# vinhisreal/YOLO-LitePi

Hardware: AMD Instinct MI355X
Metric: images/sec end-to-end (det+NMS+clf) 640x640 batch64 (higher is better)
Workload: dtype f16; 1 GPU; configs[2]: full det+NMS+ROI+ShuffleNetV2 pipeline, fp16, batch=64/GPU, 640x640, inputs resident in HBM; classifier=ShuffleNetV2 x1.0, 91 classes, seeded random weights, 64x64 ROIs, min_area=50, max_det=300, steps_in_flight=3, distinct_input_batches=4, global_batch=64, boxes_pre_area_filter_rank0=413

## Files before the change

yolo-litepi_amd/csrc/c2f_kernels.hip:

```cpp
#include "c2f.h"

#include <cstdlib>

namespace lp {

typedef _Float16 half_t;
typedef _Float16 half8 __attribute__((ext_vector_type(8)));
typedef _Float16 half4 __attribute__((ext_vector_type(4)));
typedef float floatx4 __attribute__((ext_vector_type(4)));
typedef uint32_t u32x4 __attribute__((ext_vector_type(4)));
typedef uint32_t u32x2 __attribute__((ext_vector_type(2)));

namespace {

constexpr int cdiv_c(int a, int b) { return (a + b - 1) / b; }
constexpr int min_c(int a, int b) { return a < b ? a : b; }
constexpr int max_c(int a, int b) { return a > b ? a : b; }
constexpr int deep_depth(int S, int NT, int PT, bool ldsw) {
  int d = 2;
  for (int t = 3; t <= 6 && t <= S; ++t)
    if ((t * (PT + (ldsw ? 0 : NT)) + (ldsw ? 2 * NT : 0) + NT * PT) * 4 <= 180) d = t;
  return d;
}

template <int C_, int NB_, int KA_, int KB_, bool UP_, int COUT_, int MODE_, int KS2_, int TH_ = 20, int NW_PERIMG = 8, bool AW_ = true, int WPS_ = 0,
          bool DEEP_ = false, int NWT_ = 0>
struct C2fCfg {
  static constexpr int C = C_, NB = NB_, KA = KA_, KB = KB_, COUT = COUT_, MODE = MODE_, KS2 = KS2_;
  static constexpr bool UP = UP_;
  static constexpr bool PERIMG = MODE_ >= 1;
  static constexpr bool XCV1 = MODE_ == -1;
  static constexpr int NW = MODE_ >= 1 ? NW_PERIMG : (NWT_ > 0 ? NWT_ : (C_ >= 32 ? 8 : 4));
  static constexpr int TH = TH_, TW = 20;
  static constexpr int F = PERIMG ? 1 : 2 * NB;
  static constexpr int LW = TW + 2 * F, LH = TH + 2 * F;
  static constexpr bool GK = C % 32 != 0 && C != 16;
  static constexpr bool DEEP = DEEP_ || GK || C == 96;
  static constexpr int PS = C % 16 != 0 ? 2 * C : 2 * C + 16;
  static constexpr bool Y01 = C == 16 && NB == 1 && MODE_ == 0;
  static constexpr int PS0 = Y01 ? 4 * C + 16 : PS;
  static constexpr int Y1OFF = Y01 ? 2 * C : 0;
  static constexpr int PLANE0 = LW * LH * PS0, PLANE = LW * LH * PS;
  static constexpr int XC = 2 * C;
  static constexpr int e_cv1 = PERIMG ? 0 : 2 * NB;
  static constexpr int e_a(int k) { return PERIMG ? 0 : 2 * (NB - k) - 1; }
  static constexpr int e_b(int k) { return PERIMG ? 0 : 2 * (NB - k) - 2; }
  static constexpr int npt(int e) { return cdiv_c((TH + 2 * e) * (TW + 2 * e), 16); }
  static constexpr int MAXT = (MODE_ >= 1 && NW_PERIMG == 4) ? 52 : 20;
  static constexpr int cap_pt(int nt, int pt) { return nt * pt > (nt == 3 ? 21 : MAXT) ? cdiv_c(pt, 2) : pt; }
  static constexpr bool W1_LDS = PERIMG;
  static constexpr int CT1 = 2 * C / 16, NT1 = W1_LDS ? CT1 : (CT1 % 3 == 0 ? 3 : min_c(CT1, 4)), CB1 = CT1 / NT1,
                       PT1 = W1_LDS ? 2 : cap_pt(NT1, cdiv_c(npt(e_cv1), NW / CB1));
  static constexpr int CTM = cdiv_c(C, 16), NTM = CTM % 3 == 0 ? 3 : min_c(CTM, 2), CBM = CTM / NTM;
  static constexpr int ptm(int e) { return cdiv_c(npt(e), NW / CBM); }
  static constexpr int CT2 = COUT / 16, NT2 = CT2 % 3 == 0 ? 3 : (CT2 >= 2 ? CT2 / 2 : 1), CB2 = CT2 / NT2, PT2 = cap_pt(NT2, cdiv_c(npt(0), NW / CB2));
  static constexpr int PT2W = cdiv_c(npt(0), NW / CB2);
  static constexpr int NTS = NTM, CBS = CBM, PTS = cdiv_c(npt(0), NW / CBS);
  static constexpr int WPS = WPS_ > 0 ? WPS_ : (NW == 4 && MODE_ >= 1 ? 1 : 2);
  static constexpr bool CV2_TAB = GK || (C == 16 && NB == 2);
  static constexpr bool CV2_LDS = C >= 32 || Y01 || CV2_TAB;
  static constexpr int K2G = Y01 ? 0 : (CV2_LDS ? NB * C : (2 + NB) * C);
  static constexpr bool AW = !PERIMG && AW_;
  static constexpr int c3_steps = GK ? cdiv_c(9 * (C / 8), 4) : (C >= 32 ? 9 * (C / 32) : 5);
  static constexpr int WB_CV1 = CT1 * cdiv_c(KA + KB, 32) * 1024, WB_M = CTM * c3_steps * 1024, WB_CV2 = CT2 * cdiv_c((2 + NB) * C, 32) * 1024;
  static constexpr int WSLOT = AW ? max_c(WB_CV1, max_c(WB_M, WB_CV2)) : 0;
  static constexpr int NT_S2 = XC / 16, PT_S2 = 2;
  static constexpr int WB_S2 = PERIMG ? NT_S2 * 9 * (KS2 / 32) * 1024 : 0;
  static constexpr int LDS_BYTES = max_c(PLANE0 + PLANE + 2 * WSLOT, WB_S2);
  static_assert(!W1_LDS || WB_CV1 <= PLANE, "cv1's fragments are staged in plane 1");
  static C2fShape shape() {
    C2fShape s;
    s.C = C; s.NB = NB; s.KA = KA; s.KB = KB; s.UP = UP ? 1 : 0; s.COUT = COUT; s.MODE = MODE; s.KS2 = KS2;
    return s;
  }
};

struct Ctx {
  int n, oy0, ox0, H, W;
  int lane, wave, g, sig, gam;
  int dbg;
  unsigned long long* st;
};
#define C2F_ISTAMP(k)                                          \
  if (cx.st && threadIdx.x == 0) {                             \
    __builtin_amdgcn_sched_barrier(0);                         \
    cx.st[(k)] = clock64();                                    \
    __builtin_amdgcn_sched_barrier(0);                         \
  }
struct Rg {
  int gy0, gx0, fy0, fx0, rh, rw, R;
  unsigned magic;
};

#define C2F_STAMP(k) \
  if (a.stamps && threadIdx.x == 0) a.stamps[(size_t)blockIdx.x * 16 + (k)] = ((k) == 0 || (k) == 15) ? wall_clock64() : clock64();

#define C2F_GLDS16(gptr, lptr)                                                                        \
  __builtin_amdgcn_global_load_lds((const void __attribute__((address_space(1)))*)(gptr),          \
                                   (void __attribute__((address_space(3)))*)(lptr), 16, 0, 0)

__device__ __forceinline__ void wg_sync() {
  asm volatile("s_waitcnt vmcnt(0) lgkmcnt(0)" ::: "memory");
  __builtin_amdgcn_s_barrier();
  asm volatile("" ::: "memory");
}

__device__ __forceinline__ floatx4 mma16(half8 a, half8 b, floatx4 c) { return __builtin_amdgcn_mfma_f32_16x16x32_f16(a, b, c, 0, 0, 0); }
__device__ __forceinline__ half8 as_h8(u32x4 v) { return __builtin_bit_cast(half8, v); }

__device__ __forceinline__ floatx4 silu4(floatx4 v, floatx4 b) {
  v = v + b;
  float nl2e = -1.4426950408889634f;
  asm("" : "+s"(nl2e));
  const floatx4 t = v * floatx4{nl2e, nl2e, nl2e, nl2e};
  floatx4 e;
#pragma unroll
  for (int i = 0; i < 4; ++i) e[i] = __builtin_amdgcn_exp2f(t[i]);
  e = e + 1.f;
#pragma unroll
  for (int i = 0; i < 4; ++i) e[i] = __builtin_amdgcn_rcpf(e[i]);
  return v * e;
}

template <class CFG> __device__ __forceinline__ Rg make_region(const Ctx& cx, int E) {
  Rg r;
  const int y0 = max(cx.oy0 - E, 0), y1 = min(cx.oy0 + CFG::TH + E, cx.H);
  const int x0 = max(cx.ox0 - E, 0), x1 = min(cx.ox0 + CFG::TW + E, cx.W);
// ... 33 lines not shown
      *reinterpret_cast<half8*>(dst + 16 * j) = q;
    }
  }
}
template <int NT> __device__ __forceinline__ void load_h(const char* src, half_t (&h)[4 * NT]) {
  if constexpr (NT == 1) {
    const half4 q = *reinterpret_cast<const half4*>(src);
#pragma unroll
    for (int i = 0; i < 4; ++i) h[i] = q[i];
  } else if constexpr (NT % 2 == 1) {
#pragma unroll
    for (int j = 0; j < NT; ++j) {
      const half4 q = *reinterpret_cast<const half4*>(src + 8 * j);
#pragma unroll
      for (int i = 0; i < 4; ++i) h[4 * j + i] = q[i];
    }
  } else {
#pragma unroll
    for (int j = 0; j < NT / 2; ++j) {
      const half8 q = *reinterpret_cast<const half8*>(src + 16 * j);
#pragma unroll
      for (int i = 0; i < 8; ++i) h[8 * j + i] = q[i];
    }
  }
}
template <int NT> __device__ __forceinline__ void to_half(const floatx4 (&v)[NT], half_t (&h)[4 * NT]) {
#pragma unroll
  for (int t = 0; t < NT; ++t)
#pragma unroll
    for (int r = 0; r < 4; ++r) h[4 * t + r] = (half_t)v[t][r];
}

template <int S, int DA, int DB, int NT, int PT, class LA, class LB, class FX>
__device__ __forceinline__ void kloop(floatx4 (&acc)[NT][PT], LA&& la, LB&& lb, FX&& fix) {
  half8 af[DA][NT], bf[DB][PT];
#pragma unroll
  for (int s = 0; s < DA - 1; ++s)
    if (s < S) la(s, af[s]);
#pragma unroll
  for (int s = 0; s < DB - 1; ++s)
    if (s < S) lb(s, bf[s]);
#pragma unroll
  for (int s = 0; s < S; ++s) {
    if (s + DA - 1 < S) la(s + DA - 1, af[(s + DA - 1) % DA]);
    if (s + DB - 1 < S) lb(s + DB - 1, bf[(s + DB - 1) % DB]);
    __builtin_amdgcn_sched_barrier(0);
    fix(s, bf[s % DB]);
#pragma unroll
    for (int t = 0; t < NT; ++t)
#pragma unroll
      for (int i = 0; i < PT; ++i) acc[t][i] = mma16(af[s % DA][t], bf[s % DB][i], acc[t][i]);
  }
}
struct NoFix {
  template <int PT> __device__ __forceinline__ void operator()(int, half8 (&)[PT]) const {}
};

template <bool LDSW> struct ASrc {
  const char* base;
  template <int NT> __device__ __forceinline__ void load(int off_bytes, int s, half8 (&af)[NT]) const {
#pragma unroll
    for (int t = 0; t < NT; ++t) af[t] = as_h8(*reinterpret_cast<const u32x4*>(base + off_bytes + (s * NT + t) * 1024));
  }
};
__device__ __forceinline__ void stage_weights(const Ctx& cx, const void* src, char* slot, int bytes, int nw) {
  const char* s = reinterpret_cast<const char*>(src) + cx.lane * 16;
  for (int p = cx.wave; p < (bytes >> 10); p += nw) C2F_GLDS16(s + p * 1024, slot + p * 1024);
}

template <class CFG, int NT, int CB, int PT, int KA, int KB, int KL0, int KL1, bool UP, bool LDSW, class EPI, int PSL0 = CFG::PS, int PSL1 = CFG::PS>
__device__ __forceinline__ void pw_phase(const Ctx& cx, const Rg& rg, const char* __restrict__ srcA, int pitchA, const char* __restrict__ srcB,
                                         int pitchB, const char* pl0, const char* pl1, const ASrc<LDSW>& wsrc, const float* __restrict__ bias,
                                         EPI&& epi, int stamp0 = -1) {
  static_assert(KA % 32 == 0 && KB % 8 == 0 && KL0 % 32 == 0 && KL1 % 16 == 0 && (KB % 32 == 0 || KL0 + KL1 == 0),
                "K segments: whole steps, except a tail of whole 8-channel groups at the very end (global srcB, or 16 channels of plane 1)");
  constexpr int SA = KA / 32, SB = cdiv_c(KB, 32), SL0 = KL0 / 32, SL1 = cdiv_c(KL1, 32), SG = SA + SB, S = SG + SL0 + SL1;
  const int tail_off = (4 * (SB - 1) + cx.gam < KB / 8) ? (SB - 1) * 64 : -cx.gam * 16;
  const int npt = (rg.R + 15) >> 4;
  const int nblk = ((npt + PT - 1) / PT) * CB;
  for (int blk = cx.wave; blk < nblk; blk += CFG::NW) {
    const int cb = blk % CB, pbk = blk / CB;
    unsigned offA[SA > 0 ? PT : 1], offB[SB > 0 ? PT : 1];
    int pb[SL0 + SL1 > 0 ? PT : 1];
#pragma unroll
    for (int i = 0; i < PT; ++i) {
      int p = (pbk * PT + i) * 16 + cx.sig;
      p = p < rg.R ? p : rg.R - 1;
      int py, px;
      pix_of(rg, p, py, px);
      const int gy = rg.gy0 + py, gx = rg.gx0 + px;
      if constexpr (SA > 0) {
        const int ya = UP ? (gy >> 1) : gy, xa = UP ? (gx >> 1) : gx;
        const int HA = UP ? (cx.H >> 1) : cx.H, WA = UP ? (cx.W >> 1) : cx.W;
        offA[i] = (unsigned)(((cx.n * HA + ya) * WA + xa) * pitchA) * 2u + (unsigned)cx.gam * 16u;
      }
      if constexpr (SB > 0) offB[i] = (unsigned)(((cx.n * cx.H + gy) * cx.W + gx) * pitchB) * 2u + (unsigned)cx.gam * 16u;
      if constexpr (SL0 + SL1 > 0) pb[i] = (rg.fy0 + py) * CFG::LW + rg.fx0 + px;
    }
    floatx4 acc[NT][PT];
#pragma unroll
    for (int t = 0; t < NT; ++t)
#pragma unroll
      for (int i = 0; i < PT; ++i) acc[t][i] = floatx4{0.f, 0.f, 0.f, 0.f};
    int woff = (cb * S * NT * 64 + cx.lane) * 16;
    asm volatile("" : "+v"(woff));
    floatx4 bv[NT];
#pragma unroll
    for (int t = 0; t < NT; ++t) bv[t] = *reinterpret_cast<const floatx4*>(bias + cb * 16 * NT + 4 * NT * cx.g + 4 * t);
    constexpr int DB = CFG::DEEP ? deep_depth(S, NT, PT, LDSW)
                                 : ((CFG::PERIMG && LDSW) ? min_c(S, 5) : (((NT * PT <= 20 && CFG::C >= 32) || (CFG::WPS == 1 && NT * PT <= 28)) ? 3 : 2));
    constexpr int DA = LDSW ? 2 : DB;
    if (stamp0 >= 0) { C2F_ISTAMP(stamp0) }
    kloop<S, DA, DB, NT, PT>(
        acc, [&](int s, half8(&af)[NT]) { wsrc.template load<NT>(woff, s, af); },
        [&](int s, half8(&bf)[PT]) {
#pragma unroll
          for (int i = 0; i < PT; ++i) {
            if (s < SA) bf[i] = as_h8(*reinterpret_cast<const u32x4*>(srcA + (size_t)offA[SA > 0 ? i : 0] + s * 64));
            else if (s < SG && KB % 32 != 0 && s == SG - 1) bf[i] = as_h8(*reinterpret_cast<const u32x4*>(srcB + (size_t)(offB[SB > 0 ? i : 0] + (unsigned)tail_off)));
            else if (s < SG) bf[i] = as_h8(*reinterpret_cast<const u32x4*>(srcB + (size_t)offB[SB > 0 ? i : 0] + (s - SA) * 64));
            else if (s < SG + SL0) bf[i] = as_h8(*reinterpret_cast<const u32x4*>(pl0 + pb[SL0 + SL1 > 0 ? i : 0] * PSL0 + cx.gam * 16 + (s - SG) * 64));
            else bf[i] = as_h8(*reinterpret_cast<const u32x4*>(pl1 + pb[SL0 + SL1 > 0 ? i : 0] * PSL1 + (KL1 % 32 ? (cx.gam & 1) : cx.gam) * 16 + (s - SG - SL0) * 64));
          }
        },
        NoFix{});
    if (stamp0 >= 0) { C2F_ISTAMP(stamp0 + 1) }
#pragma unroll
    for (int i = 0; i < PT; ++i) {
      const int p0 = (pbk * PT + i) * 16 + cx.sig;
      const bool ok = p0 < rg.R;
      const int p = ok ? p0 : rg.R - 1;
      int py, px;
      pix_of(rg, p, py, px);
      floatx4 v[NT];
#pragma unroll
      for (int t = 0; t < NT; ++t) v[t] = silu4(acc[t][i], bv[t]);
      epi(cb, ok, py, px, v);
    }
    if (stamp0 >= 0) { C2F_ISTAMP(stamp0 + 2) }
  }
}

template <class CFG, int NT, int CB, int PT, bool LDSW, class EPI>
__device__ __forceinline__ void pw_gk_phase(const Ctx& cx, const Rg& rg, const char* __restrict__ cat, int cat_pitch, const char* pl0, const char* pl1,
                                            const ASrc<LDSW>& wsrc, const float* __restrict__ bias, EPI&& epi, int stamp0 = -1) {
  constexpr int G0 = CFG::K2G / 8, GC = CFG::C / 8, GT = G0 + 2 * GC, S = cdiv_c(GT, 4), PS = CFG::PS;
  static_assert(CFG::PS0 == CFG::PS && G0 >= 1, "one pixel pitch for both planes; y0 comes from the concat buffer");
  int goff[S];
  const char* lbase[S];
  bool isg[S];
#pragma unroll
  for (int s = 0; s < S; ++s) {
    int q = 4 * s + cx.gam;
    q = q < GT ? q : GT - 1;
    isg[s] = q < G0;
    goff[s] = (q < G0 ? q : G0 - 1) * 16;
    const int ql = q < G0 ? 0 : q - G0;
    lbase[s] = ql < GC ? pl0 + ql * 16 : pl1 + (ql - GC) * 16;
  }
  const int npt = (rg.R + 15) >> 4;
  const int nblk = ((npt + PT - 1) / PT) * CB;
  for (int blk = cx.wave; blk < nblk; blk += CFG::NW) {
    const int cb = blk % CB, pbk = blk / CB;
    unsigned offB[PT];
    int pb[PT];
#pragma unroll
    for (int i = 0; i < PT; ++i) {
      int p = (pbk * PT + i) * 16 + cx.sig;
      p = p < rg.R ? p : rg.R - 1;
      int py, px;
      pix_of(rg, p, py, px);
      offB[i] = (unsigned)(((cx.n * cx.H + rg.gy0 + py) * cx.W + rg.gx0 + px) * cat_pitch) * 2u;
      pb[i] = ((rg.fy0 + py) * CFG::LW + rg.fx0 + px) * PS;
    }
    floatx4 acc[NT][PT];
#pragma unroll
    for (int t = 0; t < NT; ++t)
#pragma unroll
      for (int i = 0; i < PT; ++i) acc[t][i] = floatx4{0.f, 0.f, 0.f, 0.f};
    int woff = (cb * S * NT * 64 + cx.lane) * 16;
    asm volatile("" : "+v"(woff));
    floatx4 bv[NT];
#pragma unroll
    for (int t = 0; t < NT; ++t) bv[t] = *reinterpret_cast<const floatx4*>(bias + cb * 16 * NT + 4 * NT * cx.g + 4 * t);
    constexpr int DB = deep_depth(S, NT, PT, LDSW);
    constexpr int DA = LDSW ? 2 : DB;
    if (stamp0 >= 0) { C2F_ISTAMP(stamp0) }
    kloop<S, DA, DB, NT, PT>(
        acc, [&](int s, half8(&af)[NT]) { wsrc.template load<NT>(woff, s, af); },
        [&](int s, half8(&bf)[PT]) {
          const bool pure_g = 4 * s + 3 < G0, pure_l = 4 * s >= G0;
// ... 394 lines not shown
  char* WS = smem + CFG::PLANE0 + CFG::PLANE;
  Ctx cx;
  cx.lane = threadIdx.x & 63;
  cx.wave = __builtin_amdgcn_readfirstlane(threadIdx.x >> 6);
  cx.g = cx.lane >> 4;
  {
    const int col = cx.lane & 15;
    cx.sig = col < 4 ? 2 * col : (col < 12 ? 2 * (col - 4) + 1 : 2 * (col - 8));
    cx.gam = ((cx.g & 1) << 1) | (cx.g >> 1);
  }
  cx.n = blockIdx.x % a.N;
  const int tile = blockIdx.x / a.N;
  const int ty = tile / a.tiles_x, tx = tile - ty * a.tiles_x;
  cx.oy0 = ty * TH; cx.ox0 = tx * TW;
  cx.H = a.H; cx.W = a.W;
  cx.st = a.stamps ? a.stamps + (size_t)blockIdx.x * 16 : nullptr;
  cx.dbg = a.debug_store;
  C2F_STAMP(0)
  C2F_STAMP(1)

  auto wslot = [&](int q) { return WS + (q & 1) * CFG::WSLOT; };
  auto stage = [&](int q) {
    if constexpr (AW) {
      if (q == 0) { if constexpr (!CFG::XCV1) stage_weights(cx, a.w[C2F_W_CV1], wslot(0), CFG::WB_CV1, CFG::NW); }
      else if (q == 2 * NB + 1) stage_weights(cx, a.w[C2F_W_CV2], wslot(q), CFG::WB_CV2, CFG::NW);
      else if (q <= 2 * NB) stage_weights(cx, a.w[C2F_W_A0 + q - 1], wslot(q), CFG::WB_M, CFG::NW);
    }
  };
  auto wsrc = [&](int q, int widx) {
    return ASrc<AW>{AW ? wslot(q) : reinterpret_cast<const char*>(a.w[widx])};
  };
  stage(0);
  stage(1);
  const char* src1 = reinterpret_cast<const char*>(a.src1);
  char* cat = reinterpret_cast<char*>(a.cat);
  const bool dbg = (a.debug_store & 1) != 0;

  if constexpr (CFG::MODE >= 1) {
    stage_weights(cx, a.w[C2F_W_S2], smem, CFG::WB_S2, CFG::NW);
    const Rg rg = make_region<CFG>(cx, 0);
    char* xo = reinterpret_cast<char*>(a.x);
    wg_sync();
    c3s2_phase<CFG, CFG::NT_S2, 1, CFG::PT_S2, true>(cx, rg, reinterpret_cast<const char*>(a.s2_in), a.s2_pitch, ASrc<true>{smem}, a.b[C2F_W_S2],
                                                     [&](int cb, bool ok, int py, int px, const floatx4(&v)[CFG::NT_S2]) {
                                                       constexpr int NT = CFG::NT_S2;
                                                       const int chb = cb * 16 * NT + 4 * NT * cx.g;
                                                       half_t h[4 * NT];
                                                       to_half<NT>(v, h);
                                                       const int gpix = (cx.n * cx.H + rg.gy0 + py) * cx.W + rg.gx0 + px;
                                                       if (ok) store_h<NT>(xo + (size_t)((unsigned)gpix * (unsigned)a.x_pitch) * 2 + chb * 2, h);
                                                     });
    wg_sync();
  }
  {
    const bool interior = !CFG::PERIMG && cx.oy0 >= F && cx.ox0 >= F && cx.oy0 + TH + F <= a.H && cx.ox0 + TW + F <= a.W;
    if constexpr (CFG::W1_LDS) stage_weights(cx, a.w[C2F_W_CV1], P1, CFG::WB_CV1, CFG::NW);
    if (!interior) {
      constexpr int NCLR = CFG::W1_LDS ? CFG::PLANE0 : CFG::PLANE0 + CFG::PLANE;
      for (int i = threadIdx.x; i < NCLR / 16; i += CFG::NW * 64) reinterpret_cast<u32x4*>(smem)[i] = u32x4{0u, 0u, 0u, 0u};
    }
  }
  wg_sync();
  C2F_STAMP(2)

  if constexpr (CFG::XCV1) {
    const Rg rg = make_region<CFG>(cx, CFG::e_cv1);
    constexpr int CG = C / 8, NTHR = CFG::NW * 64, NPC = cdiv_c(LW * CFG::LH * CG, NTHR);
    u32x4 v[NPC];
    int dst[NPC];
#pragma unroll
    for (int j = 0; j < NPC; ++j) {
      const int it = threadIdx.x + j * NTHR;
      const int pix = it / CG, cg = it - pix * CG;
      const bool valid = pix < rg.R;
      int py, px;
      pix_of(rg, valid ? pix : rg.R - 1, py, px);
      const int gpix = (cx.n * cx.H + rg.gy0 + py) * cx.W + rg.gx0 + px;
      v[j] = *reinterpret_cast<const u32x4*>(cat + (size_t)((unsigned)gpix * (unsigned)a.cat_pitch) * 2 + C * 2 + cg * 16);
      dst[j] = valid ? ((rg.fy0 + py) * LW + rg.fx0 + px) * PS0 + Y1OFF + cg * 16 : -1;
    }
#pragma unroll
    for (int j = 0; j < NPC; ++j)
      if (dst[j] >= 0) *reinterpret_cast<u32x4*>(P0 + dst[j]) = v[j];
  } else {
    const Rg rg = make_region<CFG>(cx, CFG::e_cv1);
    pw_phase<CFG, CFG::NT1, CFG::CB1, CFG::PT1, CFG::KA, CFG::KB, 0, 0, CFG::UP, AW || CFG::W1_LDS>(
        cx, rg, reinterpret_cast<const char*>(a.src0), a.pitch0, src1, a.pitch1, nullptr, nullptr,
        ASrc < AW || CFG::W1_LDS > {CFG::W1_LDS ? P1 : (AW ? wslot(0) : reinterpret_cast<const char*>(a.w[C2F_W_CV1]))}, a.b[C2F_W_CV1],
        [&](int cb, bool ok, int py, int px, const floatx4(&v)[CFG::NT1]) {
          constexpr int NT = CFG::NT1;
          const int chb = cb * 16 * NT + 4 * NT * cx.g;
          half_t h[4 * NT];
          to_half<NT>(v, h);
          const int fy = rg.fy0 + py, fx = rg.fx0 + px;
          if (ok) {
            if (CFG::Y01) store_h<NT>(P0 + (fy * LW + fx) * PS0 + chb * 2, h);
            else if (chb >= C) store_h<NT>(P0 + (fy * LW + fx) * PS0 + (chb - C) * 2, h);
            if ((chb < CFG::K2G || dbg) && fy >= F && fy < F + TH && fx >= F && fx < F + TW) {
              const int gpix = (cx.n * cx.H + rg.gy0 + py) * cx.W + rg.gx0 + px;
              store_h<NT>(cat + (size_t)((unsigned)gpix * (unsigned)a.cat_pitch) * 2 + chb * 2, h);
            }
          }
        }, CFG::PERIMG ? -1 : 8);
  }
  wg_sync();
  if constexpr (CFG::W1_LDS) {
    for (int i = threadIdx.x; i < CFG::PLANE / 16; i += CFG::NW * 64) reinterpret_cast<u32x4*>(P1)[i] = u32x4{0u, 0u, 0u, 0u};
    lds_sync();
  }
  C2F_STAMP(3)

#pragma unroll
  for (int k = 0; k < NB; ++k) {
    stage(2 * k + 2);
    {
      const Rg rg = make_region<CFG>(cx, CFG::e_a(k));
      auto epi_a = [&](int cb, bool ok, int py, int px, const floatx4(&v)[CFG::NTM]) {
        constexpr int NT = CFG::NTM;
        const int chb = cb * 16 * NT + 4 * NT * cx.g;
        half_t h[4 * NT];
        to_half<NT>(v, h);
        if (ok && (C % 16 == 0 || chb < C)) store_h<NT>(P1 + ((rg.fy0 + py) * LW + rg.fx0 + px) * PS + chb * 2, h);
      };
      const ASrc<AW> wa = wsrc(2 * k + 1, C2F_W_A0 + 2 * k);
      const float* ba = a.b[C2F_W_A0 + 2 * k];
      if (k == 0) c3_phase<CFG, CFG::ptm(CFG::e_a(0)), false, AW, PS0, Y1OFF>(cx, rg, P0, wa, ba, epi_a);
      else c3_phase<CFG, CFG::ptm(CFG::e_a(NB - 1)), false, AW, PS0, Y1OFF>(cx, rg, P0, wa, ba, epi_a);
    }
    wg_sync();
    stage(2 * k + 3);
    {
      const Rg rg = make_region<CFG>(cx, CFG::e_b(k));
      const bool last = k == NB - 1;
      auto epi_b = [&](int cb, bool ok, int py, int px, const floatx4(&v)[CFG::NTM]) {
        constexpr int NT = CFG::NTM;
        const int chb0 = cb * 16 * NT + 4 * NT * cx.g;
        const bool real = C % 16 == 0 || chb0 < C;
        const int chb = real ? chb0 : 0;
        const int fy = rg.fy0 + py, fx = rg.fx0 + px;
        char* yp = P0 + (fy * LW + fx) * PS0 + Y1OFF + chb * 2;
        half_t r[4 * NT], h[4 * NT];
        load_h<NT>(yp, r);
#pragma unroll
        for (int t = 0; t < NT; ++t)
#pragma unroll
          for (int q = 0; q < 4; ++q) h[4 * t + q] = (half_t)((float)(half_t)v[t][q] + (float)r[4 * t + q]);
        if (ok && real) {
          if (!last) store_h<NT>(yp, h);
          else if (CFG::CV2_LDS) store_h<NT>(P1 + (fy * LW + fx) * PS + chb * 2, h);
          if (((2 + k) * C < CFG::K2G || dbg) && fy >= F && fy < F + TH && fx >= F && fx < F + TW) {
            const int gpix = (cx.n * cx.H + rg.gy0 + py) * cx.W + rg.gx0 + px;
            store_h<NT>(cat + (size_t)((unsigned)gpix * (unsigned)a.cat_pitch) * 2 + ((2 + k) * C + chb) * 2, h);
          }
        }
      };
      const ASrc<AW> wbk = wsrc(2 * k + 2, C2F_W_B0 + 2 * k);
      const float* bbk = a.b[C2F_W_B0 + 2 * k];
      if (k == 0 && NB > 1) c3_phase<CFG, CFG::ptm(CFG::e_b(0)), false, AW, PS, 0>(cx, rg, P1, wbk, bbk, epi_b);
// ... 439 lines not shown
      half_t h[4 * NT];
      to_half<NT>(v, h);
      const int chb = os * CFG::COUTW + cb * 16 * NT + 4 * NT * cx.g;
      const int gpix = (cx.n * cx.H + py) * cx.W + px;
      if (ok) store_h<NT>(out + (size_t)((unsigned)gpix * (unsigned)a.out2_pitch) * 2 + chb * 2, h);
    }
  }
}
typedef SpCfg<96, 192, 192, 2> SpCfgV2;

typedef C2fCfg<32, 1, 128, 64, true, 64, 0, 0> CfgNeck40;
typedef C2fCfg<16, 1, 64, 32, true, 32, 0, 0, 16> CfgNeck80;
typedef C2fCfg<32, 1, 0, 128, false, 64, 0, 0> CfgPan40;
typedef C2fCfg<64, 1, 0, 256, false, 128, 1, 64> CfgPan20;
typedef C2fCfg<64, 1, 0, 128, false, 128, 2, 64> CfgBb20;
typedef C2fCfg<16, 2, 0, 32, false, 32, 0, 0, 16> CfgBb80;
typedef C2fCfg<32, 2, 0, 64, false, 64, 0, 0> CfgBb40;
typedef C2fCfg<48, 1, 192, 96, true, 96, 0, 0, 20, 8, false> CfgV2Neck40;
typedef C2fCfg<48, 1, 0, 144, false, 96, 0, 0, 20, 8, false> CfgV2Pan40;
typedef C2fCfg<24, 1, 96, 48, true, 48, 0, 0, 16> CfgV2Neck80;
typedef C2fCfg<96, 1, 0, 192, false, 192, 0, 0, 10, 8, false> CfgV2Bb20;
typedef C2fCfg<96, 1, 0, 288, false, 192, 0, 0, 10, 8, false> CfgV2Pan20;
typedef C2fCfg<24, 2, 0, 48, false, 48, -1, 0, 20, 8, true, 0, false, 8> CfgV2Bb80x;
typedef C2fCfg<16, 2, 0, 32, false, 32, -1, 0, 16> CfgBb80x;
typedef C2fCfg<64, 1, 0, 256, false, 128, 0, 0, 10, 8, false> CfgPan20h;
typedef C2fCfg<64, 1, 0, 128, false, 128, 0, 0, 10, 8, false> CfgBb20h;
typedef C2fCfg<24, 2, 0, 48, false, 48, 0, 0, 20, 8, true, 0, false, 8> CfgV2Bb80;
typedef C2fCfg<48, 2, 0, 96, false, 96, 0, 0, 10, 8, false> CfgV2Bb40;

template <class CFG> struct CfgName;
#define C2F_NAME(T, s) \
  template <> struct CfgName<T> { static const char* get() { return s; } };
C2F_NAME(CfgNeck40, "c2f<32,1,up128+64>")
C2F_NAME(CfgNeck80, "c2f<16,1,up64+32>")
C2F_NAME(CfgPan40, "c2f<32,1,128>")
C2F_NAME(CfgPan20, "c2f<64,1,s2+256>")
C2F_NAME(CfgBb20, "c2f<64,1,s2+128,sppf>")
C2F_NAME(CfgBb80, "c2f<16,2,32>")
C2F_NAME(CfgBb40, "c2f<32,2,64>")
C2F_NAME(CfgV2Neck40, "c2f<48,1,up192+96>")
C2F_NAME(CfgV2Pan40, "c2f<48,1,144>")
C2F_NAME(CfgV2Neck80, "c2f<24,1,up96+48>")
C2F_NAME(CfgV2Bb20, "c2f<96,1,192>")
C2F_NAME(CfgV2Pan20, "c2f<96,1,288>")
C2F_NAME(CfgV2Bb80, "c2f<24,2,48>")
C2F_NAME(CfgBb80x, "c2f<16,2,y0y1>")
C2F_NAME(CfgV2Bb80x, "c2f<24,2,y0y1>")
C2F_NAME(CfgPan20h, "c2f<64,1,256>")
C2F_NAME(CfgBb20h, "c2f<64,1,128>")
C2F_NAME(CfgV2Bb40, "c2f<48,2,96>")

template <class CFG> size_t cfg_lds() { return (size_t)CFG::LDS_BYTES; }

template <class CFG> bool try_launch(const C2fShape& s, const C2fArgs& a, hipStream_t st) {
  if (!(s == CFG::shape())) return false;
  const size_t lds = cfg_lds<CFG>();
  set_max_dynamic_lds(reinterpret_cast<const void*>(&c2f_kernel<CFG>), (int)lds);
  const int grid = a.N * a.tiles_x * a.tiles_y;
  LP_LAUNCH(c2f_kernel<CFG>, dim3(grid), dim3(CFG::NW * 64), lds, st, a);
  return true;
}
struct CfgInfo { size_t lds; const char* name; bool perimg, gk, cv2_lds; int th, tw, nt1, ntm, nt2, nt_s2; };
template <class CFG> bool try_info(const C2fShape& s, CfgInfo& ci) {
  if (!(s == CFG::shape())) return false;
  ci.lds = cfg_lds<CFG>();
  ci.name = CfgName<CFG>::get();
  ci.perimg = CFG::PERIMG;
  ci.gk = CFG::GK;
  ci.cv2_lds = CFG::CV2_LDS;
  ci.th = CFG::TH; ci.tw = CFG::TW;
  ci.nt1 = CFG::NT1; ci.ntm = CFG::NTM; ci.nt2 = CFG::NT2; ci.nt_s2 = CFG::NT_S2;
  return true;
}
template <class F> bool for_each_cfg(F&& f) {
  return f.template operator()<CfgNeck40>() || f.template operator()<CfgNeck80>() || f.template operator()<CfgPan40>() ||
         f.template operator()<CfgPan20>() || f.template operator()<CfgBb20>() || f.template operator()<CfgBb80>() ||
         f.template operator()<CfgBb40>() || f.template operator()<CfgV2Neck40>() || f.template operator()<CfgV2Pan40>() ||
         f.template operator()<CfgV2Neck80>() || f.template operator()<CfgV2Bb20>() || f.template operator()<CfgV2Pan20>() ||
         f.template operator()<CfgV2Bb80>() || f.template operator()<CfgV2Bb40>() || f.template operator()<CfgPan20h>() ||
         f.template operator()<CfgBb20h>() || f.template operator()<CfgBb80x>() || f.template operator()<CfgV2Bb80x>();
}
struct InfoFn {
  const C2fShape& s; CfgInfo& ci;
  template <class CFG> bool operator()() const { return try_info<CFG>(s, ci); }
};
struct LaunchFn {
  const C2fShape& s; const C2fArgs& a; hipStream_t st;
  template <class CFG> bool operator()() const { return try_launch<CFG>(s, a, st); }
};
bool cfg_info(const C2fShape& s, CfgInfo& ci) { return for_each_cfg(InfoFn{s, ci}); }
bool cfg_enabled(const C2fShape& s, CfgInfo& ci) {
  if (!getenv("LITEPI_C2F_BB80") && s == CfgBb80::shape()) return false;
  if (!cfg_info(s, ci)) return false;
  if (const char* skip = getenv("LITEPI_C2F_SKIP")) {
    const std::string list = std::string(";") + skip + ";", key = std::string(";") + ci.name + ";";
    if (list.find(key) != std::string::npos) return false;
  }
  return true;
}

int gam_of(int g) { return ((g & 1) << 1) | (g >> 1); }

template <class KIDX>
void pack_phase(DevBuf& dst, const std::vector<float>& Wm, int cout, int ktot, int NT, int S, KIDX&& kidx) {
  LP_CHECK((int)Wm.size() == cout * ktot, LP_ERR_STATE, "c2f: weight matrix %zu != %d x %d", Wm.size(), cout, ktot);
  const int CB = (cout + 16 * NT - 1) / (16 * NT);
  std::vector<uint16_t> buf((size_t)CB * S * NT * 64 * 8, 0);
  for (int cb = 0; cb < CB; ++cb)
    for (int s = 0; s < S; ++s)
      for (int t = 0; t < NT; ++t)
        for (int lane = 0; lane < 64; ++lane) {
          const int g = lane >> 4, m = lane & 15, gm = m >> 2, r = m & 3;
          const int oc = cb * 16 * NT + gm * 4 * NT + t * 4 + r;
          const size_t f = ((((size_t)cb * S + s) * NT + t) * 64 + lane) * 8;
          if (oc >= cout) continue;
          for (int j = 0; j < 8; ++j) {
            const int k = kidx(s, g, j);
            if (k >= 0) buf[f + j] = f32_to_f16(Wm[(size_t)oc * ktot + k]);
          }
        }
  dst.alloc(buf.size() * 2, false);
  LP_HIP(hipMemcpy(dst.p, buf.data(), buf.size() * 2, hipMemcpyHostToDevice));
}
void put_bias(DevBuf& dst, const std::vector<float>* b, int cout) {
  std::vector<float> v(cout + 64, 0.f);
  if (b) {
    LP_CHECK((int)b->size() >= cout, LP_ERR_STATE, "c2f: bias vector too short");
    for (int c = 0; c < cout; ++c) v[c] = (*b)[c];
  }
  dst.alloc(v.size() * 4, false);
  LP_HIP(hipMemcpy(dst.p, v.data(), v.size() * 4, hipMemcpyHostToDevice));
}

}

static DevBuf g_stamp_buf;
static unsigned long long* stamp_buffer(size_t nwg) {
  if (g_stamp_buf.bytes < nwg * 16 * 8) g_stamp_buf.alloc(nwg * 16 * 8);
  LP_HIP(hipMemset(g_stamp_buf.p, 0, nwg * 16 * 8));
  return g_stamp_buf.as<unsigned long long>();
}
// ... 221 lines not shown
  a.N = N; a.H = H; a.W = W; a.tiles_x = a.tiles_y = 1;
  typedef SpCfgV2 CFG;
  set_max_dynamic_lds(reinterpret_cast<const void*>(&sppf_kernel<CFG>), CFG::LDS_BYTES);
  LP_LAUNCH(sppf_kernel<CFG>, dim3(N * CFG::OSPLIT), dim3(CFG::NW * 64), CFG::LDS_BYTES, st, a);
  LP_HIP(hipGetLastError());
}

bool C2fLayer::cv2_from_lds() const {
  CfgInfo ci;
  return cfg_info(sh, ci) && ci.cv2_lds;
}

std::string C2fLayer::kernel_name() const {
  CfgInfo ci;
  return cfg_info(sh, ci) ? ci.name : "c2f";
}

void C2fLayer::launch(const IO& io, int N, hipStream_t st) const {
  C2fArgs a;
  memset(&a, 0, sizeof(a));
  auto span_ok = [&](const View& v, int mult) { return !v.base || (double)N * v.H * v.W * v.pitch * 2.0 * mult < 4294967296.0; };
  LP_CHECK(span_ok(io.src0, 1) && span_ok(io.src1, 1) && span_ok(io.cat, 1) && span_ok(io.out, 1) && span_ok(io.s2_in, 1) && span_ok(io.x, 1) &&
               span_ok(io.cat2, 1) && span_ok(io.out2, 1), LP_ERR_ARG, "c2f: tensor too large for 32-bit byte offsets");
  LP_CHECK(io.src1.base && io.cat.base && io.out.base && io.src1.H == H && io.src1.W == W && io.cat.H == H && io.out.H == H, LP_ERR_STATE,
           "c2f %s: bad views", name.c_str());
  LP_CHECK((sh.KA > 0) == (io.src0.base != nullptr), LP_ERR_STATE, "c2f %s: src0 mismatch", name.c_str());
  if (sh.KA > 0) LP_CHECK(io.src0.H == (sh.UP ? H / 2 : H) && io.src0.W == (sh.UP ? W / 2 : W) && io.src0.C >= sh.KA, LP_ERR_STATE, "c2f %s: src0 shape", name.c_str());
  LP_CHECK(io.src1.C >= sh.KB && io.cat.C >= (2 + sh.NB) * sh.C && io.out.C >= sh.COUT, LP_ERR_STATE, "c2f %s: view channels", name.c_str());
  a.src0 = io.src0.base; a.pitch0 = io.src0.pitch;
  a.src1 = io.src1.base; a.pitch1 = io.src1.pitch;
  a.cat = io.cat.base; a.cat_pitch = io.cat.pitch;
  a.out = io.out.base; a.out_pitch = io.out.pitch;
  for (int i = 0; i < C2F_NW; ++i) { a.w[i] = d_w[i].p; a.b[i] = d_b[i].as<float>(); }
  if (sh.MODE >= 1) {
    LP_CHECK(io.s2_in.base && io.x.base && io.s2_in.H == 2 * H && io.s2_in.W == 2 * W && io.s2_in.C >= sh.KS2 && io.x.C >= 2 * sh.C, LP_ERR_STATE,
             "c2f %s: entry conv views", name.c_str());
    a.s2_in = io.s2_in.base; a.s2_pitch = io.s2_in.pitch;
    a.x = io.x.base; a.x_pitch = io.x.pitch;
  }
  if (sh.MODE == 2) {
    LP_CHECK(io.cat2.base && io.out2.base && io.cat2.C >= 4 * sh.C && io.out2.C >= sh.COUT, LP_ERR_STATE, "c2f %s: SPPF views", name.c_str());
    a.cat2 = io.cat2.base; a.cat2_pitch = io.cat2.pitch;
    a.out2 = io.out2.base; a.out2_pitch = io.out2.pitch;
  }
  a.N = N; a.H = H; a.W = W;
  CfgInfo ci;
  LP_CHECK(cfg_info(sh, ci), LP_ERR_STATE, "c2f %s: no configuration for this shape", name.c_str());
  a.tiles_x = W / ci.tw; a.tiles_y = H / ci.th;
  static const bool store_all = getenv("LITEPI_C2F_STORE_ALL") != nullptr;
  static const int dbg_flags = getenv("LITEPI_C2F_DEBUG") ? atoi(getenv("LITEPI_C2F_DEBUG")) : 0;
  a.debug_store = (store_all ? 1 : 0) | (dbg_flags & ~1);
  static const char* stamp_file = getenv("LITEPI_C2F_STAMPS");
  if (stamp_file) a.stamps = stamp_buffer((size_t)N * a.tiles_x * a.tiles_y);
  const bool ok = for_each_cfg(LaunchFn{sh, a, st});
  LP_CHECK(ok, LP_ERR_STATE, "c2f %s: no kernel for this shape", name.c_str());
  LP_HIP(hipGetLastError());
  if (stamp_file && getenv("LITEPI_C2F_TWICE")) for_each_cfg(LaunchFn{sh, a, st});
  if (stamp_file) dump_stamps(stamp_file, name, (size_t)N * a.tiles_x * a.tiles_y, st);
}

}
```

Baseline: 128,800 images/sec.

## Split upsampled cv1 into low-res partial GEMM plus skip-input GEMM

For non-per-image C2f configs with a 2x upsampled input, cv1 now first computes the upsampled-source part of the GEMM once per low-resolution pixel and stores the partial sums in LDS plane 1. Each full-resolution pixel then reads its partial sum and adds only the skip-input channels. This removes the fourfold redundant MMA work and loads on the upsampled channels. The cost is an extra LDS scratch round-trip, a workgroup barrier, and an extra plane clear on border tiles. An env var keeps the old direct path available.

```diff
diff --git a/yolo-litepi_amd/csrc/c2f_kernels.hip b/yolo-litepi_amd/csrc/c2f_kernels.hip
--- a/yolo-litepi_amd/csrc/c2f_kernels.hip
+++ b/yolo-litepi_amd/csrc/c2f_kernels.hip
@@ -68,11 +68,20 @@
   static constexpr int WB_S2 = PERIMG ? NT_S2 * 9 * (KS2 / 32) * 1024 : 0;
   static constexpr int LDS_BYTES = max_c(PLANE0 + PLANE + 2 * WSLOT, WB_S2);
   static_assert(!W1_LDS || WB_CV1 <= PLANE, "cv1's fragments are staged in plane 1");
+  static constexpr bool UP2 = UP && !PERIMG;
+  static constexpr int SCR_SRC = (LH / 2) * (LW / 2), SCR_PIX = SCR_SRC + (24 - SCR_SRC % 16) % 16, SCR_BYTES = UP2 ? XC * 4 * SCR_PIX : 0;
+  static constexpr int PT1U = cdiv_c(cdiv_c(SCR_SRC, 16), NW / CB1);
+  static_assert(!UP2 || (TH % 2 == 0 && TW % 2 == 0 && F % 2 == 0 && SCR_BYTES <= PLANE && KA > 0 && NW % CB1 == 0),
+                "two-stage cv1: even tile origins, the partial sums fit plane 1");
   static C2fShape shape() {
     C2fShape s;
     s.C = C; s.NB = NB; s.KA = KA; s.KB = KB; s.UP = UP ? 1 : 0; s.COUT = COUT; s.MODE = MODE; s.KS2 = KS2;
     return s;
   }
+};
+
+template <class CFG> struct UpDirect : CFG {
+  static constexpr bool UP2 = false;
 };
 
 struct Ctx {
@@ -212,6 +221,28 @@
       for (int i = 0; i < PT; ++i) acc[t][i] = mma16(af[s % DA][t], bf[s % DB][i], acc[t][i]);
   }
 }
+template <int S, int DA, int DB, int NT, int PT, class LA, class LB>
+__device__ __forceinline__ void kloop_pro(half8 (&af)[DA][NT], half8 (&bf)[DB][PT], LA&& la, LB&& lb) {
+#pragma unroll
+  for (int s = 0; s < DA - 1; ++s)
+    if (s < S) la(s, af[s]);
+#pragma unroll
+  for (int s = 0; s < DB - 1; ++s)
+    if (s < S) lb(s, bf[s]);
+}
+template <int S, int DA, int DB, int NT, int PT, class LA, class LB>
+__device__ __forceinline__ void kloop_main(floatx4 (&acc)[NT][PT], half8 (&af)[DA][NT], half8 (&bf)[DB][PT], LA&& la, LB&& lb) {
+#pragma unroll
+  for (int s = 0; s < S; ++s) {
+    if (s + DA - 1 < S) la(s + DA - 1, af[(s + DA - 1) % DA]);
+    if (s + DB - 1 < S) lb(s + DB - 1, bf[(s + DB - 1) % DB]);
+    __builtin_amdgcn_sched_barrier(0);
+#pragma unroll
+    for (int t = 0; t < NT; ++t)
+#pragma unroll
+      for (int i = 0; i < PT; ++i) acc[t][i] = mma16(af[s % DA][t], bf[s % DB][i], acc[t][i]);
+  }
+}
 struct NoFix {
   template <int PT> __device__ __forceinline__ void operator()(int, half8 (&)[PT]) const {}
 };
@@ -226,6 +257,11 @@
 __device__ __forceinline__ void stage_weights(const Ctx& cx, const void* src, char* slot, int bytes, int nw) {
   const char* s = reinterpret_cast<const char*>(src) + cx.lane * 16;
   for (int p = cx.wave; p < (bytes >> 10); p += nw) C2F_GLDS16(s + p * 1024, slot + p * 1024);
+}
+
+template <class CFG> constexpr int pw_depth(int S, int NT, int PT, bool ldsw) {
+  return CFG::DEEP ? deep_depth(S, NT, PT, ldsw)
+                   : ((CFG::PERIMG && ldsw) ? min_c(S, 5) : (((NT * PT <= 20 && CFG::C >= 32) || (CFG::WPS == 1 && NT * PT <= 28)) ? 3 : 2));
 }
 
 template <class CFG, int NT, int CB, int PT, int KA, int KB, int KL0, int KL1, bool UP, bool LDSW, class EPI, int PSL0 = CFG::PS, int PSL1 = CFG::PS>
@@ -267,8 +303,7 @@
     floatx4 bv[NT];
 #pragma unroll
     for (int t = 0; t < NT; ++t) bv[t] = *reinterpret_cast<const floatx4*>(bias + cb * 16 * NT + 4 * NT * cx.g + 4 * t);
-    constexpr int DB = CFG::DEEP ? deep_depth(S, NT, PT, LDSW)
-                                 : ((CFG::PERIMG && LDSW) ? min_c(S, 5) : (((NT * PT <= 20 && CFG::C >= 32) || (CFG::WPS == 1 && NT * PT <= 28)) ? 3 : 2));
+    constexpr int DB = pw_depth<CFG>(S, NT, PT, LDSW);
     constexpr int DA = LDSW ? 2 : DB;
     if (stamp0 >= 0) { C2F_ISTAMP(stamp0) }
     kloop<S, DA, DB, NT, PT>(
@@ -297,6 +332,148 @@
       for (int t = 0; t < NT; ++t) v[t] = silu4(acc[t][i], bv[t]);
       epi(cb, ok, py, px, v);
     }
+    if (stamp0 >= 0) { C2F_ISTAMP(stamp0 + 2) }
+  }
+}
+
+template <class CFG, int NT, int CB, int PT, int PTU, int KA, int KB, bool LDSW, class EPI>
+__device__ __forceinline__ void pw_up_phase(const Ctx& cx, const Rg& rg, const char* __restrict__ srcA, int pitchA, const char* __restrict__ srcB,
+                                            int pitchB, char* scr, const ASrc<LDSW>& wsrc, const float* __restrict__ bias, EPI&& epi, int stamp0 = -1) {
+  static_assert(KA % 32 == 0 && KA > 0 && KB % 8 == 0 && KB > 0, "K segments: whole steps of srcA, then srcB with a tail of whole 8-channel groups");
+  constexpr int SA = KA / 32, SB = cdiv_c(KB, 32), S = SA + SB, NSP = CFG::SCR_PIX;
+  const int sy0 = rg.gy0 >> 1, sx0 = rg.gx0 >> 1;
+  const int rhs = ((rg.gy0 + rg.rh - 1) >> 1) - sy0 + 1, rws = ((rg.gx0 + rg.rw - 1) >> 1) - sx0 + 1, RS = rhs * rws;
+  const int tail_off = (4 * (SB - 1) + cx.gam < KB / 8) ? (SB - 1) * 64 : -cx.gam * 16;
+  const int npt2 = (rg.R + 15) >> 4;
+  const int nblk2 = ((npt2 + PT - 1) / PT) * CB;
+  auto setup2 = [&](int pbk, unsigned(&offB)[PT], int(&so)[PT]) {
+#pragma unroll
+    for (int i = 0; i < PT; ++i) {
+      int p = (pbk * PT + i) * 16 + cx.sig;
+      p = p < rg.R ? p : rg.R - 1;
+      int py, px;
+      pix_of(rg, p, py, px);
+      const int gy = rg.gy0 + py, gx = rg.gx0 + px;
+      offB[i] = (unsigned)(((cx.n * cx.H + gy) * cx.W + gx) * pitchB) * 2u + (unsigned)cx.gam * 16u;
+      so[i] = (cx.g * NSP + ((gy >> 1) - sy0) * rws + (gx >> 1) - sx0) << 4;
+    }
+  };
+  auto load_b2 = [&](int s, const unsigned(&offB)[PT], half8(&bf)[PT]) {
+#pragma unroll
+    for (int i = 0; i < PT; ++i) {
+      if (KB % 32 != 0 && s == SB - 1) bf[i] = as_h8(*reinterpret_cast<const u32x4*>(srcB + (size_t)(offB[i] + (unsigned)tail_off)));
+      else bf[i] = as_h8(*reinterpret_cast<const u32x4*>(srcB + (size_t)offB[i] + s * 64));
+    }
+  };
+  auto finish2 = [&](int cb, int pbk, floatx4(&acc)[NT][PT], const floatx4(&bv)[NT]) {
+#pragma unroll
+    for (int i = 0; i < PT; ++i) {
+      const int p0 = (pbk * PT + i) * 16 + cx.sig;
+      const bool ok = p0 < rg.R;
+      const int p = ok ? p0 : rg.R - 1;
+      int py, px;
+      pix_of(rg, p, py, px);
+      floatx4 v[NT];
+#pragma unroll
+      for (int t = 0; t < NT; ++t) v[t] = silu4(acc[t][i], bv[t]);
+      epi(cb, ok, py, px, v);
+    }
+  };
+  constexpr int DB2F = SB + 1, DA2F = 2;
+  const bool has0 = cx.wave < nblk2;
+  const int cb0 = has0 ? cx.wave % CB : 0, pbk0 = has0 ? cx.wave / CB : 0;
+  int so0[PT];
+  half8 af0[DA2F][NT], bf0[DB2F][PT];
+  int woff0 = (cb0 * S * NT * 64 + cx.lane) * 16;
+  asm volatile("" : "+v"(woff0));
+  if (has0) {
+    unsigned offB0[PT];
+    setup2(pbk0, offB0, so0);
+    kloop_pro<SB, DA2F, DB2F, NT, PT>(
+        af0, bf0, [&](int s, half8(&af)[NT]) { wsrc.template load<NT>(woff0, SA + s, af); }, [&](int s, half8(&bf)[PT]) { load_b2(s, offB0, bf); });
+  }
+  {
+    const unsigned smagic = 0xFFFFFFFFu / (unsigned)rws + 1u;
+    const int HA = cx.H >> 1, WA = cx.W >> 1;
+    const int npt = (RS + 15) >> 4;
+    const int nblk = ((npt + PTU - 1) / PTU) * CB;
+    for (int blk = cx.wave; blk < nblk; blk += CFG::NW) {
+      const int cb = blk % CB, pbk = blk / CB;
+      unsigned offA[PTU];
+#pragma unroll
+      for (int i = 0; i < PTU; ++i) {
+        int p = (pbk * PTU + i) * 16 + cx.sig;
+        p = p < RS ? p : RS - 1;
+        const int py = (int)__umulhi((unsigned)p, smagic), px = p - py * rws;
+        offA[i] = (unsigned)(((cx.n * HA + sy0 + py) * WA + sx0 + px) * pitchA) * 2u + (unsigned)cx.gam * 16u;
+      }
+      floatx4 acc[NT][PTU];
+#pragma unroll
+      for (int t = 0; t < NT; ++t)
+#pragma unroll
+        for (int i = 0; i < PTU; ++i) acc[t][i] = floatx4{0.f, 0.f, 0.f, 0.f};
+      int woff = (cb * S * NT * 64 + cx.lane) * 16;
+      asm volatile("" : "+v"(woff));
+      constexpr int DB = min_c(SA + 1, LDSW ? 7 : 5);
+      constexpr int DA = LDSW ? 2 : 3;
+      kloop<SA, DA, DB, NT, PTU>(
+          acc, [&](int s, half8(&af)[NT]) { wsrc.template load<NT>(woff, s, af); },
+          [&](int s, half8(&bf)[PTU]) {
+#pragma unroll
+            for (int i = 0; i < PTU; ++i) bf[i] = as_h8(*reinterpret_cast<const u32x4*>(srcA + (size_t)offA[i] + s * 64));
+          },
+          NoFix{});
+#pragma unroll
+      for (int i = 0; i < PTU; ++i) {
+        const int p0 = (pbk * PTU + i) * 16 + cx.sig;
+        if (p0 < RS) {
+#pragma unroll
+          for (int t = 0; t < NT; ++t) *reinterpret_cast<floatx4*>(scr + ((((cb * NT + t) * 4 + cx.g) * NSP + p0) << 4)) = acc[t][i];
+        }
+      }
+    }
+  }
+  asm volatile("s_waitcnt lgkmcnt(0)" ::: "memory");
+  __builtin_amdgcn_s_barrier();
+  asm volatile("" ::: "memory");
+  if (has0) {
+    floatx4 acc[NT][PT];
+#pragma unroll
+    for (int t = 0; t < NT; ++t)
+#pragma unroll
+      for (int i = 0; i < PT; ++i) acc[t][i] = *reinterpret_cast<const floatx4*>(scr + so0[i] + (((cb0 * NT + t) * 4 * NSP) << 4));
+    floatx4 bv[NT];
+#pragma unroll
+    for (int t = 0; t < NT; ++t) bv[t] = *reinterpret_cast<const floatx4*>(bias + cb0 * 16 * NT + 4 * NT * cx.g + 4 * t);
+    if (stamp0 >= 0) { C2F_ISTAMP(stamp0) }
+    kloop_main<SB, DA2F, DB2F, NT, PT>(
+        acc, af0, bf0, [&](int s, half8(&af)[NT]) { wsrc.template load<NT>(woff0, SA + s, af); }, [&](int, half8(&)[PT]) {});
+    if (stamp0 >= 0) { C2F_ISTAMP(stamp0 + 1) }
+    finish2(cb0, pbk0, acc, bv);
+    if (stamp0 >= 0) { C2F_ISTAMP(stamp0 + 2) }
+  }
+  for (int blk = cx.wave + CFG::NW; blk < nblk2; blk += CFG::NW) {
+    const int cb = blk % CB, pbk = blk / CB;
+    unsigned offB[PT];
+    int so[PT];
+    setup2(pbk, offB, so);
+    floatx4 acc[NT][PT];
+#pragma unroll
+    for (int t = 0; t < NT; ++t)
+#pragma unroll
+      for (int i = 0; i < PT; ++i) acc[t][i] = *reinterpret_cast<const floatx4*>(scr + so[i] + (((cb * NT + t) * 4 * NSP) << 4));
+    int woff = (cb * S * NT * 64 + cx.lane) * 16;
+    asm volatile("" : "+v"(woff));
+    floatx4 bv[NT];
+#pragma unroll
+    for (int t = 0; t < NT; ++t) bv[t] = *reinterpret_cast<const floatx4*>(bias + cb * 16 * NT + 4 * NT * cx.g + 4 * t);
+    constexpr int DB = pw_depth<CFG>(SB, NT, PT, LDSW);
+    constexpr int DA = LDSW ? 2 : DB;
+    if (stamp0 >= 0) { C2F_ISTAMP(stamp0) }
+    kloop<SB, DA, DB, NT, PT>(
+        acc, [&](int s, half8(&af)[NT]) { wsrc.template load<NT>(woff, SA + s, af); }, [&](int s, half8(&bf)[PT]) { load_b2(s, offB, bf); }, NoFix{});
+    if (stamp0 >= 0) { C2F_ISTAMP(stamp0 + 1) }
+    finish2(cb, pbk, acc, bv);
     if (stamp0 >= 0) { C2F_ISTAMP(stamp0 + 2) }
   }
 }
@@ -797,11 +974,11 @@
                                                      });
     wg_sync();
   }
+  const bool interior = !CFG::PERIMG && cx.oy0 >= F && cx.ox0 >= F && cx.oy0 + TH + F <= a.H && cx.ox0 + TW + F <= a.W;
   {
-    const bool interior = !CFG::PERIMG && cx.oy0 >= F && cx.ox0 >= F && cx.oy0 + TH + F <= a.H && cx.ox0 + TW + F <= a.W;
     if constexpr (CFG::W1_LDS) stage_weights(cx, a.w[C2F_W_CV1], P1, CFG::WB_CV1, CFG::NW);
     if (!interior) {
-      constexpr int NCLR = CFG::W1_LDS ? CFG::PLANE0 : CFG::PLANE0 + CFG::PLANE;
+      constexpr int NCLR = (CFG::W1_LDS || CFG::UP2) ? CFG::PLANE0 : CFG::PLANE0 + CFG::PLANE;
       for (int i = threadIdx.x; i < NCLR / 16; i += CFG::NW * 64) reinterpret_cast<u32x4*>(smem)[i] = u32x4{0u, 0u, 0u, 0u};
     }
   }
@@ -829,10 +1006,7 @@
       if (dst[j] >= 0) *reinterpret_cast<u32x4*>(P0 + dst[j]) = v[j];
   } else {
     const Rg rg = make_region<CFG>(cx, CFG::e_cv1);
-    pw_phase<CFG, CFG::NT1, CFG::CB1, CFG::PT1, CFG::KA, CFG::KB, 0, 0, CFG::UP, AW || CFG::W1_LDS>(
-        cx, rg, reinterpret_cast<const char*>(a.src0), a.pitch0, src1, a.pitch1, nullptr, nullptr,
-        ASrc < AW || CFG::W1_LDS > {CFG::W1_LDS ? P1 : (AW ? wslot(0) : reinterpret_cast<const char*>(a.w[C2F_W_CV1]))}, a.b[C2F_W_CV1],
-        [&](int cb, bool ok, int py, int px, const floatx4(&v)[CFG::NT1]) {
+    auto epi_cv1 = [&](int cb, bool ok, int py, int px, const floatx4(&v)[CFG::NT1]) {
           constexpr int NT = CFG::NT1;
           const int chb = cb * 16 * NT + 4 * NT * cx.g;
           half_t h[4 * NT];
@@ -846,9 +1020,25 @@
               store_h<NT>(cat + (size_t)((unsigned)gpix * (unsigned)a.cat_pitch) * 2 + chb * 2, h);
             }
           }
-        }, CFG::PERIMG ? -1 : 8);
+        };
+    if constexpr (CFG::UP2) {
+      pw_up_phase<CFG, CFG::NT1, CFG::CB1, CFG::PT1, CFG::PT1U, CFG::KA, CFG::KB, AW>(
+          cx, rg, reinterpret_cast<const char*>(a.src0), a.pitch0, src1, a.pitch1, P1,
+          ASrc<AW>{AW ? wslot(0) : reinterpret_cast<const char*>(a.w[C2F_W_CV1])}, a.b[C2F_W_CV1], epi_cv1, 8);
+    } else {
+      pw_phase<CFG, CFG::NT1, CFG::CB1, CFG::PT1, CFG::KA, CFG::KB, 0, 0, CFG::UP, AW || CFG::W1_LDS>(
+          cx, rg, reinterpret_cast<const char*>(a.src0), a.pitch0, src1, a.pitch1, nullptr, nullptr,
+          ASrc < AW || CFG::W1_LDS > {CFG::W1_LDS ? P1 : (AW ? wslot(0) : reinterpret_cast<const char*>(a.w[C2F_W_CV1]))}, a.b[C2F_W_CV1],
+          epi_cv1, CFG::PERIMG ? -1 : 8);
+    }
   }
   wg_sync();
+  if constexpr (CFG::UP2) {
+    if (!interior) {
+      for (int i = threadIdx.x; i < CFG::PLANE / 16; i += CFG::NW * 64) reinterpret_cast<u32x4*>(P1)[i] = u32x4{0u, 0u, 0u, 0u};
+      lds_sync();
+    }
+  }
   if constexpr (CFG::W1_LDS) {
     for (int i = threadIdx.x; i < CFG::PLANE / 16; i += CFG::NW * 64) reinterpret_cast<u32x4*>(P1)[i] = u32x4{0u, 0u, 0u, 0u};
     lds_sync();
@@ -1394,12 +1584,20 @@
 
 template <class CFG> size_t cfg_lds() { return (size_t)CFG::LDS_BYTES; }
 
-template <class CFG> bool try_launch(const C2fShape& s, const C2fArgs& a, hipStream_t st) {
-  if (!(s == CFG::shape())) return false;
+template <class CFG> void launch_cfg(const C2fArgs& a, hipStream_t st) {
   const size_t lds = cfg_lds<CFG>();
   set_max_dynamic_lds(reinterpret_cast<const void*>(&c2f_kernel<CFG>), (int)lds);
   const int grid = a.N * a.tiles_x * a.tiles_y;
   LP_LAUNCH(c2f_kernel<CFG>, dim3(grid), dim3(CFG::NW * 64), lds, st, a);
+}
+template <class CFG> bool try_launch(const C2fShape& s, const C2fArgs& a, hipStream_t st, bool up_direct) {
+  if (!(s == CFG::shape())) return false;
+  if constexpr (CFG::UP2) {
+    if (up_direct) launch_cfg<UpDirect<CFG>>(a, st);
+    else launch_cfg<CFG>(a, st);
+  } else {
+    launch_cfg<CFG>(a, st);
+  }
   return true;
 }
 struct CfgInfo { size_t lds; const char* name; bool perimg, gk, cv2_lds; int th, tw, nt1, ntm, nt2, nt_s2; };
@@ -1427,8 +1625,8 @@
   template <class CFG> bool operator()() const { return try_info<CFG>(s, ci); }
 };
 struct LaunchFn {
-  const C2fShape& s; const C2fArgs& a; hipStream_t st;
-  template <class CFG> bool operator()() const { return try_launch<CFG>(s, a, st); }
+  const C2fShape& s; const C2fArgs& a; hipStream_t st; bool up_direct;
+  template <class CFG> bool operator()() const { return try_launch<CFG>(s, a, st, up_direct); }
 };
 bool cfg_info(const C2fShape& s, CfgInfo& ci) { return for_each_cfg(InfoFn{s, ci}); }
 bool cfg_enabled(const C2fShape& s, CfgInfo& ci) {
@@ -1756,10 +1954,11 @@
   a.debug_store = (store_all ? 1 : 0) | (dbg_flags & ~1);
   static const char* stamp_file = getenv("LITEPI_C2F_STAMPS");
   if (stamp_file) a.stamps = stamp_buffer((size_t)N * a.tiles_x * a.tiles_y);
-  const bool ok = for_each_cfg(LaunchFn{sh, a, st});
+  static const bool up_direct = getenv("LITEPI_C2F_UP_DIRECT") != nullptr;
+  const bool ok = for_each_cfg(LaunchFn{sh, a, st, up_direct});
   LP_CHECK(ok, LP_ERR_STATE, "c2f %s: no kernel for this shape", name.c_str());
   LP_HIP(hipGetLastError());
-  if (stamp_file && getenv("LITEPI_C2F_TWICE")) for_each_cfg(LaunchFn{sh, a, st});
+  if (stamp_file && getenv("LITEPI_C2F_TWICE")) for_each_cfg(LaunchFn{sh, a, st, up_direct});
   if (stamp_file) dump_stamps(stamp_file, name, (size_t)N * a.tiles_x * a.tiles_y, st);
 }
 
```

After: 129,800 images/sec (median of 6 runs). No clear change (+0.8%).
